# scrubbbbs/cbird

Measured on AMD Instinct MI355X. Metric: Hamming comparisons/sec + images hashed/sec, 1M-image index, 1/2/4/8 MI355X, higher is better.
Workload: dtype u64 hashes as 64 x FP4 signs, f32 accumulate (find, exact) / u8+f32 (hash)

## Files before the change

### cbird_amd/csrc/hamm64_mfma.hip

```cpp
#include <algorithm>
#include <mutex>
#include <vector>

#include "cbh_internal.h"
#include "fp4_sign.h"

namespace cbh {
namespace {

typedef _Float16 h2 __attribute__((ext_vector_type(2)));
typedef unsigned v4u_t __attribute__((ext_vector_type(4)));

constexpr int kThreads = 256;
constexpr int kWaves = 4;
constexpr int kHT = 8;
constexpr int kG = 2;
constexpr int e8m0(int e) { return (int)((uint32_t)(127 + e) * 0x01010101u); }

constexpr uint32_t kNeedlePad = 384;
constexpr uint32_t kNeedleBytes = 80;
struct NeedleScratch {
  uint32_t nq_pad;
  __host__ __device__ constexpr uint32_t words() const { return 0u; }
  __host__ __device__ constexpr uint32_t fold() const { return 2u * nq_pad; }
  __host__ __device__ constexpr uint32_t pre48() const { return 3u * nq_pad; }
  __host__ __device__ constexpr uint32_t pre16() const { return pre48() + nq_pad / 128u * 192u; }
  __host__ __device__ constexpr uint32_t total() const { return pre16() + nq_pad / 128u * 64u; }
};
static_assert(kNeedlePad % 64u == 0 && kNeedlePad % 96u == 0 && kNeedlePad % 128u == 0,
              "whole pairs, triples and quadruples of needle tiles");
static_assert(NeedleScratch{kNeedlePad}.total() * 16u == kNeedlePad * kNeedleBytes &&
                  NeedleScratch{5u * kNeedlePad}.total() * 16u == 5u * kNeedlePad * kNeedleBytes,
              "the regions add up to kNeedleBytes per padded needle");

__global__ __launch_bounds__(256) void k_expand_needles(const uint64_t* __restrict__ q, uint32_t nq,
                                                        uint32_t nq_pad, uint4* __restrict__ qx) {
  const uint32_t i = blockIdx.x * 256u + threadIdx.x;
  const NeedleScratch L{nq_pad};
  if (i >= L.total()) return;
  const uint32_t* w = reinterpret_cast<const uint32_t*>(q);
  if (i < L.fold()) {
    qx[i] = fp4_expand32((i >> 1) < nq ? w[i] : 0u);
  } else if (i < L.pre48()) {
    const uint32_t j = i - L.fold();
    qx[i] = fp4_expand32(j < nq ? w[2u * j] ^ w[2u * j + 1u] : 0u);
  } else if (i < L.pre16()) {
    const uint32_t u = i - L.pre48(), quad = u / 192u, m = (u % 192u) >> 6, c = u & 31u, kb = (u >> 5) & 1u;
    uint2 o[2];
#pragma unroll
    for (uint32_t k = 0; k < 2; ++k) {
      const uint32_t s = 2u * (2u * m + kb) + k, j = quad * 128u + (s / 3u) * 32u + c;
      const uint32_t lo = j < nq ? w[2u * j] : 0u, hi = j < nq ? w[2u * j + 1u] : 0u;
      o[k] = fp4_expand16(pre48_sub(lo, hi, s % 3u), s == 3u || s == 7u || s == 9u ? kFp4Four : kFp4Half);
    }
    qx[i] = make_uint4(o[0].x, o[0].y, o[1].x, o[1].y);
  } else {
    const uint32_t u = i - L.pre16(), c = u & 31u, kb = (u >> 5) & 1u;
    const uint32_t j0 = (u >> 6) * 128u + kb * 64u + c, j1 = j0 + 32u;
    const uint2 lo = fp4_expand16(j0 < nq ? fold16(w[2u * j0], w[2u * j0 + 1u]) : 0u, kFp4Half);
    const uint2 hi = fp4_expand16(j1 < nq ? fold16(w[2u * j1], w[2u * j1 + 1u]) : 0u, kFp4Four);
    qx[i] = make_uint4(lo.x, lo.y, hi.x, hi.y);
  }
}

__device__ __forceinline__ uint32_t as_u32(float f) { return __builtin_bit_cast(uint32_t, f); }
__device__ __forceinline__ void wave_order() {
  asm volatile("" ::: "memory");
  __builtin_amdgcn_wave_barrier();
  asm volatile("" ::: "memory");
}
__device__ __forceinline__ uint32_t wave_rank(uint64_t m, uint32_t base = 0u) {
  return __builtin_amdgcn_mbcnt_hi((uint32_t)(m >> 32), __builtin_amdgcn_mbcnt_lo((uint32_t)m, base));
}
__device__ __forceinline__ uint32_t cd_row(uint32_t g, uint32_t lane) { return (g & 3u) + 8u * (g >> 2) + 4u * (lane >> 5); }

struct HitParams {
  uint32_t thresh, n, nq, keep0;
  const uint64_t* q;
  const uint32_t* ids;
  cbh_record* rec;
  unsigned long long cap;
  unsigned long long* total;
  const uint2* hay;
  const uint2* qmask;
};

constexpr uint32_t kOutCap = 128;
__device__ __forceinline__ void out_flush(uint32_t* s_out, uint32_t& nout, const HitParams& hp) {
  if (nout == 0) return;
  wave_order();
  const uint32_t lane = threadIdx.x & 63u;
  unsigned long long base = 0;
  if (lane == 0) base = atomicAdd(hp.total, (unsigned long long)nout);
  const uint32_t blo = (uint32_t)__builtin_amdgcn_readfirstlane((int)(uint32_t)base);
  const uint32_t bhi = (uint32_t)__builtin_amdgcn_readfirstlane((int)(uint32_t)(base >> 32));
  base = ((unsigned long long)bhi << 32) | blo;
  for (uint32_t k = lane; k < nout; k += 64u) {
    const uint2 r = *reinterpret_cast<const uint2*>(&s_out[2u * k]);
    if (base + k < hp.cap) hp.rec[base + k] = ((cbh_record)r.y << 32) | r.x;
  }
  wave_order();
  nout = 0;
}
__device__ __forceinline__ void out_push(uint32_t* s_out, uint32_t& nout, bool has, uint32_t qidx, uint32_t dist,
                                         uint32_t id, const HitParams& hp) {
  const uint64_t m = __builtin_amdgcn_ballot_w64(has);
  if (m == 0) return;
  const uint32_t c = (uint32_t)__popcll(m);
  if (nout + c > kOutCap) out_flush(s_out, nout, hp);
  if (has) *reinterpret_cast<uint2*>(&s_out[2u * wave_rank(m, nout)]) = make_uint2(id, (qidx << 7) | dist);
  nout += c;
}

__device__ __forceinline__ bool mask_ok(const HitParams& hp, uint32_t row, uint32_t qi, uint64_t nv) {
  if (!hp.qmask) return true;
  const uint2 hv = hp.hay[row], mk = hp.qmask[qi];
  return (((hv.x ^ (uint32_t)nv) & mk.x) | ((hv.y ^ (uint32_t)(nv >> 32)) & mk.y)) == 0;
}
__device__ __forceinline__ void out_match(uint32_t* s_out, uint32_t& nout, bool under, uint32_t row, uint32_t qi,
                                          uint64_t nv, uint32_t dist, const HitParams& hp) {
  bool has = false;
  uint32_t id = 0;
  if (under && row < hp.n && mask_ok(hp, row, qi, nv)) {
    id = hp.ids[row];
    has = id != 0 || hp.keep0;
  }
  out_push(s_out, nout, has, qi, dist, id, hp);
}

template <int N, class Step>
__device__ __forceinline__ void needle_loop(const uint4* base, uint32_t voff, uint32_t nsteps, uint32_t last, Step&& step) {
  const __amdgpu_buffer_rsrc_t rsrc = __builtin_amdgcn_make_buffer_rsrc(const_cast<uint4*>(base), 0, (int)0xffffffffu, 0x27000);
  auto load = [&](uint32_t s, uint4 (&o)[N]) __attribute__((always_inline)) {
#pragma unroll
    for (uint32_t m = 0; m < (uint32_t)N; ++m) {
      const v4u_t v = __builtin_amdgcn_raw_buffer_load_b128(rsrc, (int)voff, (int)(min(s * N + m, last) * 1024u), 0);
      o[m] = make_uint4(v.x, v.y, v.z, v.w);
    }
  };
  uint4 x[N], y[N];
  load(0, x);
#pragma unroll 1
  for (uint32_t s = 0; s < nsteps; s += 2) {
    load(min(s + 1, nsteps - 1), y);
    step(s, x);
    if (s + 1 < nsteps) {
      load(min(s + 2, nsteps - 1), x);
      step(s + 1, y);
    }
  }
}
constexpr uint32_t kNoClamp = 0xffffffffu;

constexpr uint32_t kFlagMaskPre = (1u << 5) | (1u << 11) | (1u << 17) | (1u << 23);
constexpr uint32_t kFieldOnes = 1u + (1u << 6) + (1u << 12) + (1u << 18);

constexpr uint32_t kPendCap = 320;
constexpr uint32_t kOutOff = 2u * kPendCap;
constexpr uint32_t kItemOff = kOutOff + 2u * kOutCap;
constexpr uint32_t kItemCap = 63u + 64u * 8u;
constexpr uint32_t kPreQueue = kItemOff + kItemCap + 1u;
static_assert(kPendCap >= 63u + (kHT / kG) * 64u, "pending list: every lane of every group of a step");
static_assert(kG == 2, "a descriptor names the two reduction chains of a group of 32 registers");

template <int A, int B, int G>
__device__ __forceinline__ uint32_t or_regs(const v16f (&c)[G]) {
  static_assert(B - A >= 3, "range");
  uint32_t o = as_u32(c[A >> 4][A & 15]) | as_u32(c[(A + 1) >> 4][(A + 1) & 15]) | as_u32(c[(A + 2) >> 4][(A + 2) & 15]);
#pragma unroll
  for (int r = A + 3; r < B; r += 2)
    o |= as_u32(c[r >> 4][r & 15]) | (r + 1 < B ? as_u32(c[(r + 1) >> 4][(r + 1) & 15]) : 0u);
  return o;
}

#define CBH_SCALED_MFMA(A, B, C, SCALE_B) __builtin_amdgcn_mfma_scale_f32_32x32x64_f8f6f4(A, B, C, 4, 4, 0, kScaleOne, 0, SCALE_B)

struct Pre32 {
  static constexpr int kTiles = kHT, kOps = 2;
  static constexpr uint32_t operands(NeedleScratch L) { return L.fold(); }
  static __device__ __forceinline__ uint32_t last_op(uint32_t n_pairs, uint32_t p0) { return n_pairs - 1u - p0; }
  static __device__ __forceinline__ v8i hay(uint2 hv, uint32_t) { return fp4_operand(fp4_expand32(hv.x ^ hv.y)); }
  static __device__ __forceinline__ uint32_t bias(uint32_t t) { return 16u + (t - 1u); }
  static __device__ __forceinline__ int scale(int m, uint32_t half) {
    return m == 0 ? (half ? e8m0(5) : e8m0(-1)) : (half ? e8m0(17) : e8m0(11));
  }
  static __device__ __forceinline__ void chain(const v8i (&a)[kTiles], int t0, const v8i (&b)[kOps], const v16f& c0,
                                               const int (&sc)[kOps], v16f (&c)[kG]) {
#pragma unroll
    for (int t = 0; t < kG; ++t) c[t] = CBH_SCALED_MFMA(a[t0 + t], b[0], c0, sc[0]);
#pragma unroll
    for (int t = 0; t < kG; ++t) c[t] = CBH_SCALED_MFMA(a[t0 + t], b[1], c[t], sc[1]);
  }
};

struct Pre48 {
  static constexpr int kTiles = 6, kOps = 3;
  static constexpr uint32_t operands(NeedleScratch L) { return L.pre48(); }
  static __device__ __forceinline__ uint32_t last_op(uint32_t, uint32_t) { return kNoClamp; }
  static __device__ __forceinline__ v8i hay(uint2 hv, uint32_t half) {
    const uint32_t e0 = pre48_sub(hv.x, hv.y, 0), e1 = pre48_sub(hv.x, hv.y, 1), e2 = pre48_sub(hv.x, hv.y, 2);
    const uint2 s0 = fp4_expand16(half ? e2 : e0, kFp4Half);
    const uint2 s1 = fp4_expand16(half ? e0 : e1, half ? kFp4Four : kFp4Half);
    const uint2 s2 = fp4_expand16(half ? e1 : e2, kFp4Half);
    const uint2 s3 = fp4_expand16(half ? e2 : e0, half ? kFp4Half : kFp4Four);
    return v8i{(int)s0.x, (int)s0.y, (int)s1.x, (int)s1.y, (int)s2.x, (int)s2.y, (int)s3.x, (int)s3.y};
  }
  static __device__ __forceinline__ uint32_t bias(uint32_t t) { return 8u + t; }
  static __device__ __forceinline__ int scale(int m, uint32_t half) {
    return m == 0 ? e8m0(1) : m == 1 ? (half ? e8m0(10) : e8m0(7)) : (half ? e8m0(19) : e8m0(13));
  }
  static __device__ __forceinline__ void chain(const v8i (&a)[kTiles], int t0, const v8i (&b)[kOps], const v16f& c0,
                                               const int (&sc)[kOps], v16f (&c)[kG]) {
#pragma unroll
    for (int m = 0; m < kOps; ++m)
#pragma unroll
      for (int t = 0; t < kG; ++t) {
        const v8i& h = a[t0 + t];
        c[t] = CBH_SCALED_MFMA((v8i{h[2 * m], h[2 * m + 1], h[2 * m + 2], h[2 * m + 3], 0, 0, 0, 0}), b[m], m ? c[t] : c0, sc[m]);
      }
  }
};

struct Pre16 {
  static constexpr int kTiles = kHT, kOps = 1;
  static constexpr uint32_t operands(NeedleScratch L) { return L.pre16(); }
  static __device__ __forceinline__ uint32_t last_op(uint32_t, uint32_t) { return kNoClamp; }
  static __device__ __forceinline__ v8i hay(uint2 hv, uint32_t) {
    const uint32_t f = fold16(hv.x, hv.y);
    const uint2 s0 = fp4_expand16(f, kFp4Half), s1 = fp4_expand16(f, kFp4Four);
    return v8i{(int)s0.x, (int)s0.y, (int)s1.x, (int)s1.y, 0, 0, 0, 0};
  }
  static __device__ __forceinline__ uint32_t bias(uint32_t t) { return 24u + (t - 1u); }
  static __device__ __forceinline__ int scale(int, uint32_t half) { return half ? e8m0(13) : e8m0(1); }
  static __device__ __forceinline__ void chain(const v8i (&a)[kTiles], int t0, const v8i (&b)[kOps], const v16f& c0,
                                               const int (&sc)[kOps], v16f (&c)[kG]) {
#pragma unroll
    for (int t = 0; t < kG; ++t) c[t] = CBH_SCALED_MFMA(a[t0 + t], b[0], c0, sc[0]);
  }
};

#define CBH_MFMA_PARAMS                                                                                              \
  const uint2 *__restrict__ hay, const uint32_t *__restrict__ ids, uint32_t n, const uint64_t *__restrict__ q,       \
      const uint4 *__restrict__ qx, uint32_t nq, uint32_t n_pairs, uint32_t pairs_per_chunk, uint32_t thresh,        \
      cbh_record *__restrict__ rec, unsigned long long cap, unsigned long long *__restrict__ total, uint32_t keep0,  \
      const uint2 *__restrict__ qmask, const uint4 *__restrict__ qf
#define CBH_MFMA_ARGS hay, ids, n, q, qx, nq, n_pairs, pairs_per_chunk, thresh, rec, cap, total, keep0, qmask, qf

template <class V>
__device__ __forceinline__ void prefilter_body(CBH_MFMA_PARAMS) {
  constexpr int HT = V::kTiles, G = kG;
  __shared__ __attribute__((aligned(16))) uint32_t s_queue_[kWaves][kPreQueue];
  __shared__ __attribute__((aligned(16))) uint2 s_hay_[kWaves][HT * 32];
  const uint32_t lane = threadIdx.x & 63u;
  const uint32_t wave = (uint32_t)__builtin_amdgcn_readfirstlane((int)(threadIdx.x >> 6));
  const uint32_t r = lane & 31u, half = lane >> 5;
  const uint32_t tile0 = (blockIdx.x * kWaves + wave) * HT;
  if (tile0 * 32u >= n) return;
  uint32_t* s_queue = s_queue_[wave];
  uint2* s_hay = s_hay_[wave];
  uint32_t* s_out = s_queue + kOutOff;
  uint32_t nout = 0;

  v8i a[HT];
#pragma unroll
  for (int t = 0; t < HT; ++t) {
    const uint32_t row = (tile0 + t) * 32u + r;
    const uint2 hv = row < n ? hay[row] : make_uint2(0u, 0u);
    a[t] = V::hay(hv, half);
    if (half == 0) s_hay[t * 32 + r] = hv;
  }
  wave_order();
  v16f c0;
#pragma unroll
  for (int g = 0; g < 16; ++g) c0[g] = 8388608.0f + (float)(V::bias(thresh) * kFieldOnes);
  asm volatile("" : "+v"(c0));
  int scale[V::kOps];
#pragma unroll
  for (int m = 0; m < V::kOps; ++m) {
    scale[m] = V::scale(m, half);
    asm volatile("" : "+v"(scale[m]));
  }

  const uint32_t p0 = blockIdx.y * pairs_per_chunk;
  const uint32_t p1 = min(n_pairs, p0 + pairs_per_chunk);
  const HitParams hp = {thresh, n, nq, keep0, q, ids, rec, cap, total, hay, qmask};

  uint32_t npend = 0;
  uint32_t nitem = 0;
  uint32_t* s_item = s_queue + kItemOff;
  auto work = [&](uint32_t idx, bool live) {
    const uint32_t it = s_item[idx];
    const uint32_t f = it & 3u, ch = (it >> 2) & 1u, L = (it >> 3) & 63u, pp = p0 + 2u * (it >> 11);
    const uint32_t row0 = ((it >> 9) & 3u) * 64u;
    const uint32_t qi = pp * 64u + (L & 31u) + 32u * f;
    const uint64_t nv = live && qi < hp.nq ? hp.q[qi] : 0;
    const uint32_t qlo = (uint32_t)nv, qhi = (uint32_t)(nv >> 32);
    const uint32_t rows = nv == 0 ? 0u : ch ? 0xfffe0000u : 0x0001ffffu;
    const uint2* hq = s_hay + row0 + cd_row(16u * ch, L);
    uint32_t hit = 0;
#pragma unroll 1
    for (uint32_t i = 0; i < 5u; ++i) {
      const uint32_t qd = 4u * ch + i;
      const uint4* h4 = reinterpret_cast<const uint4*>(hq + 8u * min(i, 4u - ch));
      const uint4 x = h4[0], y = h4[1];
      const uint32_t d0 = __popc(x.x ^ qlo) + __popc(x.y ^ qhi), d1 = __popc(x.z ^ qlo) + __popc(x.w ^ qhi);
      const uint32_t d2 = __popc(y.x ^ qlo) + __popc(y.y ^ qhi), d3 = __popc(y.z ^ qlo) + __popc(y.w ^ qhi);
      const uint32_t m4 = (d0 < hp.thresh ? 1u : 0u) | (d1 < hp.thresh ? 2u : 0u) | (d2 < hp.thresh ? 4u : 0u) |
                          (d3 < hp.thresh ? 8u : 0u);
      hit |= qd < 8u ? m4 << (4u * qd) : 0u;
    }
    hit &= rows;
    while (__builtin_amdgcn_ballot_w64(hit != 0) != 0) {
      const uint32_t wr = row0 + cd_row((uint32_t)__builtin_ctz(hit | 0x80000000u), L);
      const uint2 hv = s_hay[wr];
      out_match(s_out, nout, hit != 0, tile0 * 32u + wr, qi, nv, __popc(hv.x ^ qlo) + __popc(hv.y ^ qhi), hp);
      hit &= hit - 1u;
    }
  };
  auto drain = [&](bool all) {
    wave_order();
    const uint32_t keep = all ? 0u : (npend & 63u);
    uint32_t k0 = keep;
    for (;;) {
      if (nitem < 64u && k0 < npend) {
        const uint2 e = *reinterpret_cast<const uint2*>(&s_queue[2u * min(k0 + lane, npend - 1u)]);
        uint32_t cm = 0;
#pragma unroll
        for (uint32_t c = 0; c < 2; ++c) {
          const uint32_t w = e.x >> c;
          cm |= (((w >> 23) & 1u) ? 0xfu : (((w >> 5) & 1u) | (((w >> 11) & 1u) << 1) | (((w >> 17) & 1u) << 2))) << (4u * c);
        }
        if (k0 + lane >= npend) cm = 0;
#pragma unroll
        for (uint32_t b = 0; b < 8; ++b) {
          const bool on = ((cm >> b) & 1u) != 0;
          const uint64_t m = __builtin_amdgcn_ballot_w64(on);
          if (on) s_item[wave_rank(m, nitem)] = (e.y << 3) | b;
          nitem += (uint32_t)__popcll(m);
        }
        k0 += 64u;
        wave_order();
        continue;
      }
      uint32_t idx;
      bool live = true;
      if (nitem >= 64u) {
        nitem -= 64u;
        idx = nitem + lane;
      } else if (all && nitem != 0) {
        idx = min(lane, nitem - 1u);
        live = lane < nitem;
        nitem = 0;
      } else {
        break;
      }
      work(idx, live);
      wave_order();
    }
    npend = keep;
  };

  auto detect = [&](const v16f (&c)[G], const uint32_t group, const uint32_t step) __attribute__((always_inline)) {
    constexpr int R = G * 16;
    constexpr int RA = R / 2 + 1;
    const uint32_t half0 = or_regs<0, RA, G>(c), half1 = or_regs<RA, R, G>(c);
    const uint32_t flags = (half0 | half1) & kFlagMaskPre;
    const uint64_t hm = __builtin_amdgcn_ballot_w64(flags != 0);
    if (hm != 0) {
      static_assert(R == 32, "two chains of 17 and 15 registers");
      uint32_t ln = lane;
      asm volatile("" : "+v"(ln));
      if (flags != 0)
        *reinterpret_cast<uint2*>(&s_queue[2u * wave_rank(hm, npend)]) =
            make_uint2((half0 & kFlagMaskPre) | ((half1 & kFlagMaskPre) << 1), ln | (group << 6) | (step << 8));
      npend += (uint32_t)__popcll(hm);
    }
  };

  needle_loop<V::kOps>(qf + (size_t)(p0 >> 1) * (V::kOps * 64u), lane * 16u, (p1 - p0 + 1u) >> 1, V::last_op(n_pairs, p0),
                       [&](const uint32_t s, const uint4 (&nn)[V::kOps]) __attribute__((always_inline)) {
    v8i b[V::kOps];
#pragma unroll
    for (int m = 0; m < V::kOps; ++m) b[m] = fp4_operand(nn[m]);
#pragma unroll
    for (int t0 = 0; t0 < HT; t0 += G) {
      v16f c[G];
      V::chain(a, t0, b, c0, scale, c);
      detect(c, (uint32_t)(t0 / G), s);
    }
    if (npend >= 64u) drain(false);
  });
  if (npend | nitem) drain(true);
  out_flush(s_out, nout, hp);
}

template <bool PRE>
__global__ void k_hamm64_mfma(CBH_MFMA_PARAMS);
template <>
__global__ __launch_bounds__(kThreads, 4) void k_hamm64_mfma<true>(CBH_MFMA_PARAMS) { prefilter_body<Pre32>(CBH_MFMA_ARGS); }
__global__ __launch_bounds__(kThreads, 3) void k_hamm64_mfma48(CBH_MFMA_PARAMS) { prefilter_body<Pre48>(CBH_MFMA_ARGS); }
__global__ __launch_bounds__(kThreads, 4) void k_hamm64_mfma16(CBH_MFMA_PARAMS) { prefilter_body<Pre16>(CBH_MFMA_ARGS); }

__device__ __forceinline__ void load_hay_words(const uint2* __restrict__ hay, uint32_t n, uint32_t tile0, v8i (&a)[kHT]) {
  const uint32_t r = threadIdx.x & 31u, half = (threadIdx.x >> 5) & 1u;
#pragma unroll
  for (int t = 0; t < kHT; ++t) {
    const uint32_t row = (tile0 + t) * 32u + r;
    const uint2 hv = row < n ? hay[row] : make_uint2(0u, 0u);
    a[t] = fp4_operand(fp4_expand32(half ? hv.y : hv.x));
  }
}

constexpr uint32_t kLoZero2 = 0x4080u, kHiZero2 = 0x4B40u;
__device__ __forceinline__ h2 as_h2(float f) { return __builtin_bit_cast(h2, f); }
__device__ __forceinline__ h2 pkmax3(h2 a, h2 b, h2 c) {
  return __builtin_elementwise_maximum(__builtin_elementwise_maximum(a, b), c);
}
__device__ __forceinline__ void handle_tile2(const v16f& c, uint32_t row0, uint32_t p, uint32_t lo_key, uint32_t hi_key,
                                             const HitParams& hp, uint32_t* s_queue, uint32_t* s_out, uint32_t& nout) {
  const uint32_t lane = threadIdx.x & 63u;
  {
    h2 m0 = {0, 0}, m1 = {0, 0};
#pragma unroll
    for (int g = 0; g < 16; g += 4) {
      m0 = pkmax3(m0, as_h2(c[g]), as_h2(c[g + 1]));
      m1 = pkmax3(m1, as_h2(c[g + 2]), as_h2(c[g + 3]));
    }
    const uint32_t tb = __builtin_bit_cast(uint32_t, __builtin_elementwise_maximum(m0, m1));
    if (__builtin_amdgcn_ballot_w64((tb << 16) >= lo_key || tb >= hi_key) == 0) return;
  }
  uint32_t cnt = 0;
#pragma unroll
  for (int g = 0; g < 16; ++g) {
    const uint32_t bits = as_u32(c[g]);
    const bool fh = bits >= hi_key;
    const bool fl = (bits << 16) >= lo_key;
    if (__builtin_amdgcn_ballot_w64(fh || fl) == 0) continue;
    const uint64_t mh = __builtin_amdgcn_ballot_w64(fh);
    if (fh) s_queue[wave_rank(mh, cnt)] = ((kHiZero2 - (bits >> 16)) << 12) | (1u << 10) | ((uint32_t)g << 6) | lane;
    cnt += (uint32_t)__popcll(mh);
    const uint64_t ml = __builtin_amdgcn_ballot_w64(fl);
    if (fl) s_queue[wave_rank(ml, cnt)] = (((kLoZero2 - (bits & 0xffffu)) >> 1) << 12) | ((uint32_t)g << 6) | lane;
    cnt += (uint32_t)__popcll(ml);
  }
  wave_order();
  for (uint32_t k0 = 0; k0 < cnt; k0 += 64u) {
    const uint32_t k = k0 + lane;
    const uint32_t e = s_queue[min(k, cnt - 1u)];
    const uint32_t src = e & 63u, g = (e >> 6) & 15u, field = (e >> 10) & 1u, d = e >> 12;
    const uint32_t row = row0 + cd_row(g, src);
    const uint32_t qi = p * 64u + field * 32u + (src & 31u);
    bool under = false;
    uint64_t nv = 0;
    if (k < cnt && row < hp.n && qi < hp.nq) {
      nv = hp.q[qi];
      under = nv != 0 && d < hp.thresh;
    }
    out_match(s_out, nout, under, row, qi, nv, d, hp);
  }
  wave_order();
}

template <>
__global__ __launch_bounds__(kThreads, 1) void k_hamm64_mfma<false>(CBH_MFMA_PARAMS) {
  constexpr int HT = kHT, G = kG;
  constexpr uint32_t kQueue = 2048;
  __shared__ uint32_t s_queue_[kWaves][kQueue];
  __shared__ uint32_t s_out_[kWaves][2 * kOutCap];
  const uint32_t lane = threadIdx.x & 63u, wave = threadIdx.x >> 6;
  const uint32_t tile0 = (blockIdx.x * kWaves + wave) * HT;
  if (tile0 * 32u >= n) return;
  uint32_t* s_queue = s_queue_[wave];
  uint32_t* s_out = s_out_[wave];
  uint32_t nout = 0;

  v8i a[HT];
  load_hay_words(hay, n, tile0, a);
  v16f c0;
#pragma unroll
  for (int g = 0; g < 16; ++g) c0[g] = 8388608.0f + 16448.0f + 2097152.0f;
  asm volatile("" : "+v"(c0));
  const uint32_t lo_key = (kLoZero2 - 2u * (thresh - 1u)) << 16, hi_key = (kHiZero2 - (thresh - 1u)) << 16;
  const HitParams hp = {thresh, n, nq, keep0, q, ids, rec, cap, total, hay, qmask};

  const uint32_t p0 = blockIdx.y * pairs_per_chunk;
  const uint32_t p1 = min(n_pairs, p0 + pairs_per_chunk);
  needle_loop<2>(qx + (size_t)p0 * 128u, (2u * (lane & 31u) + (lane >> 5)) * 16u, p1 - p0, kNoClamp,
                 [&](const uint32_t s, const uint4 (&nn)[2]) __attribute__((always_inline)) {
    const v8i bA = fp4_operand(nn[0]), bB = fp4_operand(nn[1]);
#pragma unroll
    for (int t0 = 0; t0 < HT; t0 += G) {
      v16f c[G];
#pragma unroll
      for (int t = 0; t < G; ++t) c[t] = CBH_SCALED_MFMA(a[t0 + t], bA, c0, kScaleOne);
#pragma unroll
      for (int t = 0; t < G; ++t) c[t] = CBH_SCALED_MFMA(a[t0 + t], bB, c[t], e8m0(15));
      h2 m0 = {0, 0}, m1 = {0, 0};
#pragma unroll
      for (int t = 0; t < G; ++t)
#pragma unroll
        for (int g = 0; g < 16; g += 4) {
          m0 = pkmax3(m0, as_h2(c[t][g]), as_h2(c[t][g + 1]));
          m1 = pkmax3(m1, as_h2(c[t][g + 2]), as_h2(c[t][g + 3]));
        }
      const uint32_t mb = __builtin_bit_cast(uint32_t, __builtin_elementwise_maximum(m0, m1));
      if (__builtin_amdgcn_ballot_w64((mb << 16) >= lo_key || mb >= hi_key) != 0) {
#pragma unroll
        for (int t = 0; t < G; ++t)
          handle_tile2(c[t], (tile0 + t0 + t) * 32u, p0 + s, lo_key, hi_key, hp, s_queue, s_out, nout);
      }
    }
  });
  out_flush(s_out, nout, hp);
}
#undef CBH_MFMA_PARAMS
#undef CBH_MFMA_ARGS

constexpr uint32_t kFlagMask3 = (1u << 7) | (1u << 14) | (1u << 21);

__device__ __forceinline__ void handle_tile3(const v16f& c, uint32_t row0, uint32_t p3, const HitParams& hp,
                                             uint32_t* s_queue, uint32_t* s_out, uint32_t& nout) {
  const uint32_t lane = threadIdx.x & 63u;
  uint32_t any = 0;
#pragma unroll
  for (int g = 0; g < 16; ++g) any |= as_u32(c[g]);
  if (__builtin_amdgcn_ballot_w64((any & kFlagMask3) != 0) == 0) return;
  const uint32_t b = hp.thresh - 1u;
#pragma unroll 1
  for (uint32_t f = 0; f < 3; ++f) {
    uint32_t cnt = 0;
#pragma unroll
    for (int g = 0; g < 16; ++g) {
      const uint32_t bits = as_u32(c[g]);
      const bool fl = (bits >> (7u + 7u * f)) & 1u;
      const uint64_t m = __builtin_amdgcn_ballot_w64(fl);
      if (m == 0) continue;
      if (fl)
        s_queue[wave_rank(m, cnt)] = ((64u + b - ((bits >> (1u + 7u * f)) & 0x7fu)) << 12) | (f << 10) | ((uint32_t)g << 6) | lane;
      cnt += (uint32_t)__popcll(m);
    }
    wave_order();
    for (uint32_t k0 = 0; k0 < cnt; k0 += 64u) {
      const uint32_t k = k0 + lane;
      const uint32_t e = s_queue[min(k, cnt - 1u)];
      const uint32_t src = e & 63u, g = (e >> 6) & 15u, field = (e >> 10) & 3u, d = e >> 12;
      const uint32_t row = row0 + cd_row(g, src);
      const uint32_t qi = p3 * 96u + field * 32u + (src & 31u);
      const uint64_t nv = (k < cnt && row < hp.n && qi < hp.nq) ? hp.q[qi] : 0;
      out_match(s_out, nout, nv != 0, row, qi, nv, d, hp);
    }
    wave_order();
  }
}

__global__ __launch_bounds__(kThreads, 2) void k_hamm64_mfma3(
    const uint2* __restrict__ hay, const uint32_t* __restrict__ ids, uint32_t n,
    const uint64_t* __restrict__ q, const uint4* __restrict__ qx, uint32_t nq, uint32_t n_triples,
    uint32_t triples_per_chunk, uint32_t thresh, cbh_record* __restrict__ rec,
    unsigned long long cap, unsigned long long* __restrict__ total, uint32_t keep0,
    const uint2* __restrict__ qmask) {
  constexpr int HT = kHT, G = kG;
  __shared__ uint32_t s_queue_[kWaves][16 * 64];
  __shared__ uint32_t s_out_[kWaves][2 * kOutCap];
  const uint32_t lane = threadIdx.x & 63u, wave = threadIdx.x >> 6;
  const uint32_t tile0 = (blockIdx.x * kWaves + wave) * HT;
  if (tile0 * 32u >= n) return;
  uint32_t* s_queue = s_queue_[wave];
  uint32_t* s_out = s_out_[wave];
  uint32_t nout = 0;

  v8i a[HT];
  load_hay_words(hay, n, tile0, a);
  const uint32_t b = thresh - 1u;
  v16f c0;
#pragma unroll
  for (int g = 0; g < 16; ++g) c0[g] = 8388608.0f + (float)((64u + 2u * b) * 16513u);
  asm volatile("" : "+v"(c0));
  const HitParams hp = {thresh, n, nq, keep0, q, ids, rec, cap, total, hay, qmask};

  const uint32_t p0 = blockIdx.y * triples_per_chunk;
  const uint32_t p1 = min(n_triples, p0 + triples_per_chunk);
  needle_loop<3>(qx + (size_t)p0 * 192u, (2u * (lane & 31u) + (lane >> 5)) * 16u, p1 - p0, kNoClamp,
                 [&](const uint32_t s, const uint4 (&nn)[3]) __attribute__((always_inline)) {
    const v8i b0 = fp4_operand(nn[0]), b1 = fp4_operand(nn[1]), b2 = fp4_operand(nn[2]);
#pragma unroll
    for (int t0 = 0; t0 < HT; t0 += G) {
      v16f c[G];
#pragma unroll
      for (int t = 0; t < G; ++t) c[t] = CBH_SCALED_MFMA(a[t0 + t], b0, c0, kScaleOne);
#pragma unroll
      for (int t = 0; t < G; ++t) c[t] = CBH_SCALED_MFMA(a[t0 + t], b1, c[t], e8m0(7));
#pragma unroll
      for (int t = 0; t < G; ++t) c[t] = CBH_SCALED_MFMA(a[t0 + t], b2, c[t], e8m0(14));
      if (__builtin_amdgcn_ballot_w64((or_regs<0, G * 16, G>(c) & kFlagMask3) != 0) != 0) {
#pragma unroll
        for (int t = 0; t < G; ++t) handle_tile3(c[t], (tile0 + t0 + t) * 32u, p0 + s, hp, s_queue, s_out, nout);
      }
    }
  });
  out_flush(s_out, nout, hp);
}

constexpr uint32_t kProbeS = 2048;
constexpr int kProbeT = kProbeMaxThresh;

__device__ __forceinline__ uint32_t probe_mix(uint32_t x) {
  x = ((x >> 16) ^ x) * 0x45d9f3bu;
  x = ((x >> 16) ^ x) * 0x45d9f3bu;
  return (x >> 16) ^ x;
}
__global__ __launch_bounds__(256) void k_fold_probe(const uint2* __restrict__ hay, uint32_t n, const uint2* __restrict__ q,
                                                    uint32_t nq, uint32_t sh, uint32_t sq, uint32_t* __restrict__ counts) {
  __shared__ uint2 s_h[64];
  __shared__ uint32_t s_cnt[4 * kProbeT];
  const uint32_t t = threadIdx.x;
  if (t < 64) {
    const uint32_t i = blockIdx.y * 64u + t;
    s_h[t] = i < sh ? hay[sh == n ? i : probe_mix(i) % n] : make_uint2(0u, 0u);
  }
  if (t < 4 * kProbeT) s_cnt[t] = 0;
  __syncthreads();
  const uint32_t j = blockIdx.x * 256u + t;
  const uint32_t nslots = min(64u, sh - blockIdx.y * 64u);
  uint32_t cnt[kProbeT] = {}, cnt64[kProbeT] = {}, cnt48[kProbeT] = {}, cnt16[kProbeT] = {};
  if (j < sq) {
    const uint2 nv = q[sq == nq ? j : probe_mix(j ^ 0x9e3779b9u) % nq];
    const uint32_t f = nv.x ^ nv.y;
    for (uint32_t k = 0; k < nslots; ++k) {
      const uint2 hv = s_h[k];
      const uint32_t d = (uint32_t)__popc(f ^ hv.x ^ hv.y);
#pragma unroll
      for (int th = 0; th < kProbeT; ++th) cnt[th] += d < (uint32_t)(th + 1) ? 1u : 0u;
      const uint32_t d48 = (uint32_t)__popc((f ^ hv.x ^ hv.y) & 0xffffu) + (uint32_t)__popc((nv.x ^ hv.x) >> 16) +
                           (uint32_t)__popc((nv.y ^ hv.y) >> 16);
#pragma unroll
      for (int th = 0; th < kProbeT; ++th) cnt48[th] += d48 <= (uint32_t)(th + 1) || d48 > (uint32_t)(th + 33) ? 1u : 0u;
      const uint32_t x32 = f ^ hv.x ^ hv.y, d16 = (uint32_t)__popc((x32 ^ (x32 >> 16)) & 0xffffu);
#pragma unroll
      for (int th = 0; th < kProbeT; ++th) cnt16[th] += d16 < (uint32_t)(th + 1) ? 1u : 0u;
      if (d < (uint32_t)kProbeT) {
        const uint32_t d64 = (uint32_t)__popc(nv.x ^ hv.x) + (uint32_t)__popc(nv.y ^ hv.y);
#pragma unroll
// ... 161 lines not shown
```

### cbird_amd/csrc/hamm64_scan.hip

```cpp
#include <atomic>

#include "cbh_internal.h"

namespace cbh {
namespace {

constexpr int kThreads = 256;
constexpr int kH = 8;
constexpr int kQB = 8;

__device__ __forceinline__ uint32_t min3u(uint32_t a, uint32_t b, uint32_t c) {
  return min(min(a, b), c);
}

__device__ __forceinline__ void emit(cbh_record* __restrict__ rec, unsigned long long cap,
                                     unsigned long long* __restrict__ total, uint32_t qidx,
                                     uint32_t dist, uint32_t id) {
  unsigned long long slot = atomicAdd(total, 1ull);
  if (slot < cap) rec[slot] = ((cbh_record)qidx << 39) | ((cbh_record)dist << 32) | id;
}

template <int H>
__device__ __forceinline__ void exact_block(const uint2 (&h)[H], uint32_t base_idx, uint32_t n,
                                            const uint32_t* __restrict__ ids,
                                            const uint64_t* __restrict__ q, uint32_t qa,
                                            uint32_t qb, uint32_t thresh,
                                            cbh_record* __restrict__ rec, unsigned long long cap,
                                            unsigned long long* __restrict__ total,
                                            uint32_t keep0, const uint2* __restrict__ qmask) {
#pragma unroll 1
  for (uint32_t qi = qa; qi < qb; ++qi) {
    const uint64_t qq = q[qi];
    if (qq == 0) continue;
    const uint32_t ql = (uint32_t)qq, qh = (uint32_t)(qq >> 32);
    const uint2 mk = qmask ? qmask[qi] : make_uint2(0u, 0u);
#pragma unroll
    for (int j = 0; j < H; ++j) {
      const uint32_t d = __popc(h[j].x ^ ql) + __popc(h[j].y ^ qh);
      if (d < thresh && (((h[j].x ^ ql) & mk.x) | ((h[j].y ^ qh) & mk.y)) == 0) {
        const uint32_t idx = base_idx + (uint32_t)j * kThreads;
        if (idx < n) {
          const uint32_t id = ids[idx];
          if (id != 0 || keep0) emit(rec, cap, total, qi, d, id);
        }
      }
    }
  }
}

template <int H, int QB>
__device__ __forceinline__ void refine_block(const uint2 (&h)[H], const uint32_t (&acc)[H],
                                             const uint2 (&cur)[QB], uint32_t base_idx, uint32_t n,
                                             const uint32_t* __restrict__ ids, uint32_t qb,
                                             uint32_t thresh, cbh_record* __restrict__ rec,
                                             unsigned long long cap,
                                             unsigned long long* __restrict__ total,
                                             uint32_t keep0, const uint2* __restrict__ qmask) {
#pragma unroll
  for (int j = 0; j < H; ++j) {
    if (acc[j] < thresh) {
      const uint32_t idx = base_idx + (uint32_t)j * kThreads;
      uint32_t d[QB];
#pragma unroll
      for (int i = 0; i < QB; ++i) d[i] = __popc(h[j].x ^ cur[i].x) + __popc(h[j].y ^ cur[i].y);
      uint32_t m = d[0];
#pragma unroll
      for (int i = 1; i + 1 < QB; i += 2) m = min3u(m, d[i], d[i + 1]);
      if (QB % 2 == 0) m = min(m, d[QB - 1]);
      if (m < thresh && idx < n) {
        const uint32_t id = ids[idx];
        if (id != 0 || keep0) {
#pragma unroll
          for (int i = 0; i < QB; ++i)
            if (d[i] < thresh && (cur[i].x | cur[i].y) != 0) {
              const uint2 mk = qmask ? qmask[qb + (uint32_t)i] : make_uint2(0u, 0u);
              if ((((h[j].x ^ cur[i].x) & mk.x) | ((h[j].y ^ cur[i].y) & mk.y)) == 0)
                emit(rec, cap, total, qb + (uint32_t)i, d[i], id);
            }
        }
      }
    }
  }
}

enum { MODE_PRE = 0, MODE_FULL = 1, MODE_EQ = 2 };

template <int H, int QB, int MODE>
__global__ __launch_bounds__(kThreads) void k_hamm64_scan(
    const uint2* __restrict__ hay, const uint32_t* __restrict__ ids, uint32_t n,
    const uint64_t* __restrict__ q, uint32_t nq, uint32_t q_chunk, uint32_t thresh,
    cbh_record* __restrict__ rec, unsigned long long cap, unsigned long long* __restrict__ total,
    uint32_t keep0, const uint2* __restrict__ qmask) {
  const uint32_t base_idx = blockIdx.x * (uint32_t)(kThreads * H) + threadIdx.x;
  uint2 h[H];
#pragma unroll
  for (int j = 0; j < H; ++j) {
    const uint32_t idx = base_idx + (uint32_t)j * kThreads;
    h[j] = idx < n ? hay[idx] : make_uint2(0u, 0u);
  }
  const uint32_t q0 = blockIdx.y * q_chunk;
  const uint32_t q1 = min(nq, q0 + q_chunk);
  uint32_t qb = q0;
  const uint2* __restrict__ qp = reinterpret_cast<const uint2*>(q) + (size_t)q0;

  uint2 cur[QB];
  if (qb + QB <= q1) {
#pragma unroll
    for (int i = 0; i < QB; ++i) cur[i] = qp[i];
  }
  for (; qb + QB <= q1; qb += QB) {
    uint2 nxt[QB];
    qp += QB;
    if (qb + 2 * QB <= q1) {
#pragma unroll
      for (int i = 0; i < QB; ++i) nxt[i] = qp[i];
    } else {
#pragma unroll
      for (int i = 0; i < QB; ++i) nxt[i] = make_uint2(0u, 0u);
    }
    if (MODE == MODE_EQ) {
      unsigned long long any = 0;
#pragma unroll
      for (int i = 0; i < QB; ++i) {
        const unsigned long long qq = ((unsigned long long)cur[i].y << 32) | cur[i].x;
#pragma unroll
        for (int j = 0; j < H; ++j) {
          const unsigned long long hh = ((unsigned long long)h[j].y << 32) | h[j].x;
          any |= __ballot(hh == qq);
        }
      }
      if (any) exact_block<H>(h, base_idx, n, ids, q, qb, qb + QB, thresh, rec, cap, total, keep0, qmask);
    } else {
      uint32_t acc[H];
#pragma unroll
      for (int j = 0; j < H; ++j) acc[j] = 0xffu;
      uint32_t ql[QB], qh[QB];
#pragma unroll
      for (int i = 0; i < QB; ++i) {
        asm volatile("v_mov_b32 %0, %1" : "=v"(ql[i]) : "s"(cur[i].x));
        if (MODE == MODE_FULL) asm volatile("v_mov_b32 %0, %1" : "=v"(qh[i]) : "s"(cur[i].y));
      }
      uint32_t x[QB][H];
      __builtin_amdgcn_sched_barrier(0);
#pragma unroll
      for (int i = 0; i < QB; ++i)
#pragma unroll
        for (int j = 0; j < H; ++j) x[i][j] = h[j].x ^ ql[i];
      __builtin_amdgcn_sched_barrier(0);
      if (MODE == MODE_FULL) {
#pragma unroll
        for (int i = 0; i < QB; ++i)
#pragma unroll
          for (int j = 0; j < H; ++j) x[i][j] = (uint32_t)__popc(x[i][j]);
        uint32_t y[QB][H];
        __builtin_amdgcn_sched_barrier(0);
#pragma unroll
        for (int i = 0; i < QB; ++i)
#pragma unroll
          for (int j = 0; j < H; ++j) y[i][j] = h[j].y ^ qh[i];
        __builtin_amdgcn_sched_barrier(0);
#pragma unroll
        for (int i = 0; i < QB; i += 2)
#pragma unroll
          for (int j = 0; j < H; ++j)
            acc[j] = min3u(acc[j], x[i][j] + (uint32_t)__popc(y[i][j]),
                           x[i + 1][j] + (uint32_t)__popc(y[i + 1][j]));
      } else {
#pragma unroll
        for (int i = 0; i < QB; i += 2)
#pragma unroll
          for (int j = 0; j < H; ++j)
            acc[j] = min3u(acc[j], (uint32_t)__popc(x[i][j]), (uint32_t)__popc(x[i + 1][j]));
      }
      __builtin_amdgcn_sched_barrier(0);
      uint32_t m = acc[0];
#pragma unroll
      for (int j = 1; j + 1 < H; j += 2) m = min3u(m, acc[j], acc[j + 1]);
      if (H % 2 == 0) m = min(m, acc[H - 1]);
      if (m < thresh) refine_block<H, QB>(h, acc, cur, base_idx, n, ids, qb, thresh, rec, cap, total, keep0, qmask);
    }
#pragma unroll
    for (int i = 0; i < QB; ++i) cur[i] = nxt[i];
  }
  if (qb < q1) exact_block<H>(h, base_idx, n, ids, q, qb, q1, thresh, rec, cap, total, keep0, qmask);
}

__global__ __launch_bounds__(256) void k_zero_needle_list(const uint64_t* __restrict__ q, uint32_t nq,
                                                          uint32_t* __restrict__ list ) {
  const uint32_t qi = blockIdx.x * 256u + threadIdx.x;
  if (qi < nq && q[qi] == 0) list[1u + atomicAdd(&list[0], 1u)] = qi;
}

__global__ __launch_bounds__(256) void k_zero_needle_scan(const uint2* __restrict__ hay, const uint32_t* __restrict__ ids,
                                                          uint32_t n, const uint32_t* __restrict__ list, uint32_t thresh,
                                                          cbh_record* __restrict__ rec, unsigned long long cap,
                                                          unsigned long long* __restrict__ total, uint32_t keep0,
                                                          const uint2* __restrict__ qmask) {
  const uint32_t i = blockIdx.x * 256u + threadIdx.x;
  const uint32_t nz = list[0];
  if (i >= n || nz == 0) return;
  const uint2 h = hay[i];
  const uint32_t d = (uint32_t)__popc(h.x) + (uint32_t)__popc(h.y);
  if (d >= thresh) return;
  const uint32_t id = ids[i];
  if (id == 0 && !keep0) return;
  for (uint32_t k = 0; k < nz; ++k) {
    const uint32_t qi = list[1u + k];
    const uint2 mk = qmask ? qmask[qi] : make_uint2(0u, 0u);
    if (((h.x & mk.x) | (h.y & mk.y)) == 0) emit(rec, cap, total, qi, d, id);
  }
}

constexpr unsigned kLoneSlots = 8;
__global__ __launch_bounds__(256) void k_find_one(const uint2* __restrict__ hay, const uint32_t* __restrict__ ids,
                                                  uint32_t n, uint32_t qlo, uint32_t qhi, uint32_t thresh,
                                                  unsigned* __restrict__ d_state, LoneBlock* __restrict__ host,
                                                  unsigned long long seq) {
  const uint32_t base = blockIdx.x * (256u * kLoneSlots) + threadIdx.x;
  bool wrote = false;
#pragma unroll
  for (unsigned k = 0; k < kLoneSlots; ++k) {
    const uint32_t i = base + k * 256u;
    if (i >= n) break;
    const uint2 hv = hay[i];
    const uint32_t d = (uint32_t)__popc(hv.x ^ qlo) + (uint32_t)__popc(hv.y ^ qhi);
    if (d < thresh) {
      const uint32_t id = ids[i];
      if (id != 0) {
        const unsigned slot = atomicAdd(&d_state[0], 1u);
        if (slot < LoneBlock::kRecs) {
          host->recs[slot] = ((cbh_record)d << 32) | id;
          wrote = true;
        }
      }
    }
  }
  if (wrote) __threadfence_system();
  __syncthreads();
  if (threadIdx.x == 0) {
    __threadfence();
    if (atomicAdd(&d_state[1], 1u) == gridDim.x - 1u) {
      __threadfence();
      host->count = atomicExch(&d_state[0], 0u);
      d_state[1] = 0u;
      __threadfence_system();
      __hip_atomic_store(const_cast<unsigned long long*>(&host->done), seq, __ATOMIC_RELEASE, __HIP_MEMORY_SCOPE_SYSTEM);
    }
  }
}

}

int launch_find_one(const uint64_t* d_hashes, const uint32_t* d_ids, size_t n, uint64_t q, int thresh, unsigned* d_state,
                    LoneBlock* h_block, unsigned long long seq, hipStream_t stream) {
  if (n == 0 || n > 0xfffffff0ull || !d_state || !h_block || thresh <= 0) return CBH_E_INVAL;
  const unsigned per_wg = 256u * kLoneSlots;
  hipLaunchKernelGGL(k_find_one, dim3((unsigned)((n + per_wg - 1) / per_wg)), dim3(256), 0, stream,
                     reinterpret_cast<const uint2*>(d_hashes), d_ids, (uint32_t)n, (uint32_t)q, (uint32_t)(q >> 32),
                     (uint32_t)thresh, d_state, h_block, seq);
  CBH_HIP(hipGetLastError());
  return CBH_OK;
}

int wait_find_one(const LoneBlock* h_block, unsigned long long seq, hipStream_t stream) {
  const unsigned long long* flag = const_cast<const unsigned long long*>(&h_block->done);
  for (unsigned spins = 0;; ++spins) {
    if (__atomic_load_n(flag, __ATOMIC_ACQUIRE) == seq) return CBH_OK;
    if ((spins & 0xfffu) == 0xfffu) {
      const hipError_t q = hipStreamQuery(stream);
      if (q == hipSuccess) {
        return __atomic_load_n(flag, __ATOMIC_ACQUIRE) == seq ? CBH_OK : CBH_E_HIP;
      }
      if (q != hipErrorNotReady) {
        set_last_error("k_find_one", q);
        return CBH_E_HIP;
      }
    }
#if defined(__x86_64__)
    __builtin_ia32_pause();
#endif
  }
}

namespace {

constexpr int kPreMax = 7;
constexpr size_t kMfmaMinNq = 256;
constexpr size_t kMfmaMinN = 4096;
constexpr int kPreStatic = 6;
constexpr double kTrueWeight = 8.0;
constexpr double kSlopePre = 1.3e4, kBaseFull = 15.75, kTrueFull = 2.7e5, kTruePre = 0.7e5;
constexpr double kBasePre = 8.55, kBase48 = 14.0, kSlope48 = 2.8e4, kTrue48 = 1.0e5, kPre48Margin = 0.9;
constexpr double kBase16 = 5.85, kPre16Margin = 0.9;
constexpr uint64_t kProbeMinPairs = 1ull << 31;

int g_scan_mfma = 1;
int g_pre_max_thresh = -1;
int g_pre_rate_max_e9 = 300000;
int g_pre48 = -1;
int g_pre16 = -1;
std::atomic<uint64_t> g_variant_mask[4];
std::atomic<uint64_t> g_n_probe{0};
std::atomic<long long> g_last_rate_e9{-1};
std::atomic<long long> g_last_true_e9{-1};
std::atomic<long long> g_last_rate48_e9{-1};
std::atomic<long long> g_last_rate16_e9{-1};

enum class Join { None, IfCheaper, Forced };
enum class Kernel { PopcEq, PopcPre, PopcFull, Mfma };
struct Route {
  Join join;
  Kernel kernel;
  double scan_ms;
};

Route route(size_t n, size_t nq, int thresh, bool masked) {
  Route r;
  const double pairs = (double)n * (double)nq;
  const double pre_ms = pairs * (thresh <= 5 ? 8.7e-12 : thresh == 6 ? 9.7e-12 : thresh == 7 ? 12.1e-12 : 15.8e-12);
  r.scan_ms = thresh == 1 ? pairs * 6.1e-12 : pre_ms;
  const bool joinable = thresh <= kJoinMaxThresh && !masked && n < 0xfffffff0ull;
  r.join = !joinable ? Join::None : g_scan_mfma == 4 ? Join::Forced
           : g_scan_mfma == 3 && pre_ms >= 1.0 ? Join::IfCheaper : Join::None;
  const bool mfma = thresh <= 65 && (g_scan_mfma == 2 || g_scan_mfma == 4 ||
                                     (g_scan_mfma != 0 && nq >= kMfmaMinNq && n >= kMfmaMinN));
  r.kernel = mfma ? Kernel::Mfma : thresh == 1 ? Kernel::PopcEq : thresh <= kPreMax ? Kernel::PopcPre : Kernel::PopcFull;
  return r;
}

void note_variant(int thresh, ScanVariant v) {
  for (int i = 1; i < 4; ++i)
    if (i == (int)v) g_variant_mask[i] |= 1ull << thresh; else g_variant_mask[i] &= ~(1ull << thresh);
}

int launch_popc(Kernel kernel, const uint64_t* d_hashes, const uint32_t* d_ids, size_t n, const uint64_t* d_q, size_t nq,
                int thresh, cbh_record* d_rec, size_t cap, unsigned long long* d_total, hipStream_t stream,
                const ScanOpts& o) {
  const uint32_t tile = kThreads * kH;
  const uint32_t tiles = (uint32_t)((n + tile - 1) / tile);
  const uint32_t q_chunk = scan_chunk(tiles, nq, 16384, 1024, kQB);
  dim3 grid(tiles, (uint32_t)((nq + q_chunk - 1) / q_chunk)), block(kThreads);
  const uint2* hay = reinterpret_cast<const uint2*>(d_hashes);
#define CBH_SCAN(MODE)                                                                                                  \
  hipLaunchKernelGGL((k_hamm64_scan<kH, kQB, MODE>), grid, block, 0, stream, hay, d_ids, (uint32_t)n, d_q, (uint32_t)nq, \
                     q_chunk, (uint32_t)thresh, d_rec, (unsigned long long)cap, d_total, (uint32_t)o.keep_id0,            \
                     reinterpret_cast<const uint2*>(o.d_qmask))
  if (kernel == Kernel::PopcEq) CBH_SCAN(MODE_EQ);
  else if (kernel == Kernel::PopcPre) CBH_SCAN(MODE_PRE);
  else CBH_SCAN(MODE_FULL);
#undef CBH_SCAN
  CBH_HIP(hipGetLastError());
  return CBH_OK;
}

}

bool scan_takes_mfma(size_t n, size_t nq, int thresh) {
  return thresh >= 1 && route(n, nq, thresh, false).kernel == Kernel::Mfma;
}

bool scan_routes_to_join(size_t n, size_t nq, int thresh, bool masked) {
  return thresh >= 1 && n >= 1 && nq >= 1 && route(n, nq, thresh, masked).join != Join::None;
}

ScanVariant scan_pick_pre(const uint64_t* d_hashes, size_t n, size_t n_total, const uint64_t* d_q, size_t nq, int thresh,
                          hipStream_t stream) {
  using V = ScanVariant;
  if (g_pre16 == 1 && thresh <= max_thresh(V::Pre16)) return V::Pre16;
  if (g_pre48 == 1 && thresh <= max_thresh(V::Pre48)) return V::Pre48;
  if (thresh > max_thresh(V::Pre32)) return V::Full;
  if (g_pre_max_thresh >= 0) return thresh <= g_pre_max_thresh ? V::Pre32 : V::Full;
  if (thresh > kProbeMaxThresh) return V::Full;
  double r_cand = 0, r_true = 0, r48 = 0, r16 = 0;
  if ((uint64_t)n_total * (uint64_t)nq < kProbeMinPairs ||
      !probe_fold_rates(d_hashes, n, d_q, nq, thresh, stream, &r_cand, &r_true, &r48, &r16))
    return thresh <= kPreStatic ? V::Pre32 : V::Full;
  g_last_rate_e9 = (long long)(r_cand * 1e9);
  g_last_true_e9 = (long long)(r_true * 1e9);
  g_last_rate48_e9 = (long long)(r48 * 1e9);
  g_last_rate16_e9 = (long long)(r16 * 1e9);
  g_n_probe++;
  const double d_pre = kSlopePre * (r_cand - kTrueWeight * r_true - (double)g_pre_rate_max_e9 * 1e-9);
  const bool pre = d_pre <= 0;
  const double t_pre = kBasePre + kSlopePre * r_cand + kTruePre * r_true, t_full = kBaseFull + kTrueFull * r_true;
  if (g_pre16 != 0 && pre && thresh <= max_thresh(V::Pre16) &&
      kBase16 + kSlopePre * r16 + kTruePre * r_true < kPre16Margin * t_pre)
    return V::Pre16;
  if (g_pre48 != 0) {
    const double t_48 = kBase48 + kSlope48 * r48 + kTrue48 * r_true;
    if (pre ? t_48 < kPre48Margin * t_pre : t_48 < t_full) return V::Pre48;
  }
  return pre ? V::Pre32 : V::Full;
}

namespace {

int launch_zero_needles(const uint64_t* d_hashes, const uint32_t* d_ids, size_t n, const uint64_t* d_q, size_t nq,
                        int thresh, cbh_record* d_rec, size_t cap, unsigned long long* d_total, hipStream_t stream,
                        const ScanOpts& o) {
  Scratch scratch(stream);
  uint32_t* list = nullptr;
  CBH_HIP(scratch.get(&list, (nq + 1) * sizeof(uint32_t)));
  CBH_HIP(hipMemsetAsync(list, 0, sizeof(uint32_t), stream));
  hipLaunchKernelGGL(k_zero_needle_list, dim3((unsigned)((nq + 255) / 256)), dim3(256), 0, stream, d_q, (uint32_t)nq, list);
  hipLaunchKernelGGL(k_zero_needle_scan, dim3((unsigned)((n + 255) / 256)), dim3(256), 0, stream,
                     reinterpret_cast<const uint2*>(d_hashes), d_ids, (uint32_t)n, list, (uint32_t)thresh, d_rec,
                     (unsigned long long)cap, d_total, (uint32_t)o.keep_id0, reinterpret_cast<const uint2*>(o.d_qmask));
  CBH_HIP(hipGetLastError());
  return CBH_OK;
}

int scan_nonzero_needles(const uint64_t* d_hashes, const uint32_t* d_ids, size_t n, const uint64_t* d_q, size_t nq,
                         int thresh, cbh_record* d_rec, size_t cap, unsigned long long* d_total, hipStream_t stream,
                         const ScanOpts& o);

}

int launch_hamm64_scan(const uint64_t* d_hashes, const uint32_t* d_ids, size_t n, const uint64_t* d_q, size_t nq,
                       int thresh, cbh_record* d_rec, size_t cap, unsigned long long* d_total, hipStream_t stream,
                       const ScanOpts& o) {
  if (n == 0 || nq == 0 || thresh <= 0) return CBH_OK;
  if (n > 0xfffffff0ull || nq > CBH_MAX_QUERIES_PER_CALL) return CBH_E_INVAL;
  const int rc = scan_nonzero_needles(d_hashes, d_ids, n, d_q, nq, thresh, d_rec, cap, d_total, stream, o);
  if (rc || !o.zero_needles) return rc;
  return launch_zero_needles(d_hashes, d_ids, n, d_q, nq, thresh, d_rec, cap, d_total, stream, o);
}

namespace {

int scan_nonzero_needles(const uint64_t* d_hashes, const uint32_t* d_ids, size_t n, const uint64_t* d_q, size_t nq,
                         int thresh, cbh_record* d_rec, size_t cap, unsigned long long* d_total, hipStream_t stream,
                         const ScanOpts& o) {
  const Route r = route(n, nq, thresh, o.d_qmask != nullptr);
  if (r.join != Join::None) {
    const bool force = r.join == Join::Forced;
    const int rc = launch_hamm64_join(d_hashes, d_ids, n, d_q, nq, thresh, d_rec, cap, d_total, stream, o, force, r.scan_ms);
    if (rc == CBH_OK || force || (rc != CBH_E_UNSUPPORTED && rc != CBH_E_NOMEM)) return rc;
    if (rc == CBH_E_NOMEM) cbh_clear_error();
  }
  if (r.kernel != Kernel::Mfma) return launch_popc(r.kernel, d_hashes, d_ids, n, d_q, nq, thresh, d_rec, cap, d_total, stream, o);
  const ScanVariant v = o.pre != ScanVariant::Auto ? o.pre : scan_pick_pre(d_hashes, n, n, d_q, nq, thresh, stream);
  if (thresh < 64) note_variant(thresh, v);
  return launch_hamm64_scan_mfma(d_hashes, d_ids, n, d_q, nq, thresh, d_rec, cap, d_total, stream, v, o);
}

}

int set_scan_mfma(int mode) {
  if (mode < 0 || mode > 4) return CBH_E_INVAL;
  g_scan_mfma = mode;
  return CBH_OK;
}
int get_scan_mfma() { return g_scan_mfma; }
void set_scan_pre_max(int t) {
  if (t >= -1 && t <= max_thresh(ScanVariant::Pre32)) g_pre_max_thresh = t;
}
void set_scan_pre_rate(int e9) {
  if (e9 >= 0) g_pre_rate_max_e9 = e9;
}
void set_scan_pre48(int v) {
  if (v >= -1 && v <= 1) g_pre48 = v;
}
long long get_scan_pre_mask() { return (long long)(g_variant_mask[(int)ScanVariant::Pre32] | g_variant_mask[(int)ScanVariant::Pre16]); }
int set_scan_pre16(int v) {
  if (v < -1 || v > 1) return CBH_E_INVAL;
  g_pre16 = v;
  return CBH_OK;
}
long long get_scan_pre48_mask() { return (long long)g_variant_mask[(int)ScanVariant::Pre48].load(); }
long long get_scan_pre16_mask() { return (long long)g_variant_mask[(int)ScanVariant::Pre16].load(); }
long long get_scan_probes() { return (long long)g_n_probe.load(); }
long long get_scan_probe_rate_e9() { return g_last_rate_e9.load(); }
long long get_scan_probe_true_e9() { return g_last_true_e9.load(); }
long long get_scan_probe_rate48_e9() { return g_last_rate48_e9.load(); }
long long get_scan_probe_rate16_e9() { return g_last_rate16_e9.load(); }

}
```

Baseline: 87760 billion.

## Filter candidate rows with folded-popcount lower bound and DPP prefix-sum item compaction

Reworks the MFMA candidate verification step. It first computes a cheap lower bound on Hamming distance, popcount of lo^hi^qfold, for all 17 rows and packs the pass/fail bits into a mask with alignbit. Only rows that survive the bound get an exact popcount check. The drain step replaces eight ballot/mbcnt rounds with one DPP wave prefix sum and per-lane serial writes, and decodes the bits with a multiply trick. Routing cost constants for the pre-filter thresholds are retuned, which may change which path is chosen and relies on the bound being valid.

New measurement: 88920 billion (median of 6 runs). 1.3% higher.

```diff
diff --git a/cbird_amd/csrc/hamm64_mfma.hip b/cbird_amd/csrc/hamm64_mfma.hip
--- a/cbird_amd/csrc/hamm64_mfma.hip
+++ b/cbird_amd/csrc/hamm64_mfma.hip
@@ -72,6 +72,15 @@
 __device__ __forceinline__ uint32_t wave_rank(uint64_t m, uint32_t base = 0u) {
   return __builtin_amdgcn_mbcnt_hi((uint32_t)(m >> 32), __builtin_amdgcn_mbcnt_lo((uint32_t)m, base));
 }
+__device__ __forceinline__ uint32_t wave_prefix_sum(uint32_t v) {
+  v += (uint32_t)__builtin_amdgcn_update_dpp(0, (int)v, 0x111, 0xf, 0xf, false);
+  v += (uint32_t)__builtin_amdgcn_update_dpp(0, (int)v, 0x112, 0xf, 0xf, false);
+  v += (uint32_t)__builtin_amdgcn_update_dpp(0, (int)v, 0x114, 0xf, 0xf, false);
+  v += (uint32_t)__builtin_amdgcn_update_dpp(0, (int)v, 0x118, 0xf, 0xf, false);
+  v += (uint32_t)__builtin_amdgcn_update_dpp(0, (int)v, 0x142, 0xa, 0xf, false);
+  v += (uint32_t)__builtin_amdgcn_update_dpp(0, (int)v, 0x143, 0xc, 0xf, false);
+  return v;
+}
 __device__ __forceinline__ uint32_t cd_row(uint32_t g, uint32_t lane) { return (g & 3u) + 8u * (g >> 2) + 4u * (lane >> 5); }
 
 struct HitParams {
@@ -294,22 +303,34 @@
     const uint32_t row0 = ((it >> 9) & 3u) * 64u;
     const uint32_t qi = pp * 64u + (L & 31u) + 32u * f;
     const uint64_t nv = live && qi < hp.nq ? hp.q[qi] : 0;
-    const uint32_t qlo = (uint32_t)nv, qhi = (uint32_t)(nv >> 32);
-    const uint32_t rows = nv == 0 ? 0u : ch ? 0xfffe0000u : 0x0001ffffu;
+    const uint32_t qlo = (uint32_t)nv, qhi = (uint32_t)(nv >> 32), qfold = qlo ^ qhi;
+    const uint32_t rows = nv == 0 ? 0u : ch ? 0x0000fffeu : 0x0001ffffu;
     const uint2* hq = s_hay + row0 + cd_row(16u * ch, L);
+    const uint32_t far0 = 0x80000000u - hp.thresh;
+    uint32_t far = 0;
+    auto shift_in = [&](uint32_t lo, uint32_t hi) __attribute__((always_inline)) {
+      far = __builtin_amdgcn_alignbit(far, (uint32_t)__popc(__builtin_amdgcn_bitop3_b32(lo, hi, qfold, 0x96)) + far0, 31u);
+    };
+    {
+      const uint2 h = hq[ch ? 0u : 32u];
+      shift_in(h.x, h.y);
+    }
+#pragma unroll
+    for (int i = 3; i >= 0; --i) {
+      const uint4* h4 = reinterpret_cast<const uint4*>(hq + 8 * i);
+      const uint4 x = h4[0], y = h4[1];
+      shift_in(y.z, y.w);
+      shift_in(y.x, y.y);
+      shift_in(x.z, x.w);
+      shift_in(x.x, x.y);
+    }
     uint32_t hit = 0;
-#pragma unroll 1
-    for (uint32_t i = 0; i < 5u; ++i) {
-      const uint32_t qd = 4u * ch + i;
-      const uint4* h4 = reinterpret_cast<const uint4*>(hq + 8u * min(i, 4u - ch));
-      const uint4 x = h4[0], y = h4[1];
-      const uint32_t d0 = __popc(x.x ^ qlo) + __popc(x.y ^ qhi), d1 = __popc(x.z ^ qlo) + __popc(x.w ^ qhi);
-      const uint32_t d2 = __popc(y.x ^ qlo) + __popc(y.y ^ qhi), d3 = __popc(y.z ^ qlo) + __popc(y.w ^ qhi);
-      const uint32_t m4 = (d0 < hp.thresh ? 1u : 0u) | (d1 < hp.thresh ? 2u : 0u) | (d2 < hp.thresh ? 4u : 0u) |
-                          (d3 < hp.thresh ? 8u : 0u);
-      hit |= qd < 8u ? m4 << (4u * qd) : 0u;
-    }
-    hit &= rows;
+    for (uint32_t sv = ~far & rows; sv != 0; sv &= sv - 1u) {
+      const uint32_t k = (uint32_t)__builtin_ctz(sv);
+      const uint2 hv = hq[k + (k & 0x1cu)];
+      if (__popc(hv.x ^ qlo) + __popc(hv.y ^ qhi) < hp.thresh) hit |= 1u << k;
+    }
+    hit <<= 16u * ch;
     while (__builtin_amdgcn_ballot_w64(hit != 0) != 0) {
       const uint32_t wr = row0 + cd_row((uint32_t)__builtin_ctz(hit | 0x80000000u), L);
       const uint2 hv = s_hay[wr];
@@ -327,17 +348,14 @@
         uint32_t cm = 0;
 #pragma unroll
         for (uint32_t c = 0; c < 2; ++c) {
-          const uint32_t w = e.x >> c;
-          cm |= (((w >> 23) & 1u) ? 0xfu : (((w >> 5) & 1u) | (((w >> 11) & 1u) << 1) | (((w >> 17) & 1u) << 2))) << (4u * c);
+          const uint32_t nb = ((((e.x >> (5u + c)) & 0x41041u) * 0x8421u) >> 15) & 0xfu;
+          cm |= (nb > 7u ? 0xfu : nb) << (4u * c);
         }
         if (k0 + lane >= npend) cm = 0;
-#pragma unroll
-        for (uint32_t b = 0; b < 8; ++b) {
-          const bool on = ((cm >> b) & 1u) != 0;
-          const uint64_t m = __builtin_amdgcn_ballot_w64(on);
-          if (on) s_item[wave_rank(m, nitem)] = (e.y << 3) | b;
-          nitem += (uint32_t)__popcll(m);
-        }
+        const uint32_t cnt = (uint32_t)__popc(cm), upto = wave_prefix_sum(cnt);
+        uint32_t* dst = s_item + nitem + (upto - cnt);
+        for (const uint32_t item0 = e.y << 3; cm != 0; cm &= cm - 1u) *dst++ = item0 | (uint32_t)__builtin_ctz(cm);
+        nitem += (uint32_t)__builtin_amdgcn_readlane((int)upto, 63);
         k0 += 64u;
         wave_order();
         continue;
diff --git a/cbird_amd/csrc/hamm64_scan.hip b/cbird_amd/csrc/hamm64_scan.hip
--- a/cbird_amd/csrc/hamm64_scan.hip
+++ b/cbird_amd/csrc/hamm64_scan.hip
@@ -289,7 +289,7 @@
 constexpr size_t kMfmaMinN = 4096;
 constexpr int kPreStatic = 6;
 constexpr double kTrueWeight = 8.0;
-constexpr double kSlopePre = 1.3e4, kBaseFull = 15.75, kTrueFull = 2.7e5, kTruePre = 0.7e5;
+constexpr double kSlopePre = 1.0e4, kBaseFull = 15.75, kTrueFull = 2.7e5, kTruePre = 0.7e5;
 constexpr double kBasePre = 8.55, kBase48 = 14.0, kSlope48 = 2.8e4, kTrue48 = 1.0e5, kPre48Margin = 0.9;
 constexpr double kBase16 = 5.85, kPre16Margin = 0.9;
 constexpr uint64_t kProbeMinPairs = 1ull << 31;
@@ -317,7 +317,7 @@
 Route route(size_t n, size_t nq, int thresh, bool masked) {
   Route r;
   const double pairs = (double)n * (double)nq;
-  const double pre_ms = pairs * (thresh <= 5 ? 8.7e-12 : thresh == 6 ? 9.7e-12 : thresh == 7 ? 12.1e-12 : 15.8e-12);
+  const double pre_ms = pairs * (thresh <= 5 ? 8.7e-12 : thresh == 6 ? 9.5e-12 : thresh == 7 ? 11.3e-12 : 15.8e-12);
   r.scan_ms = thresh == 1 ? pairs * 6.1e-12 : pre_ms;
   const bool joinable = thresh <= kJoinMaxThresh && !masked && n < 0xfffffff0ull;
   r.join = !joinable ? Join::None : g_scan_mfma == 4 ? Join::Forced
```
